# ctu-mrs/mrs_uav_trajectory_generation

Measured on AMD Instinct MI355X. Metric: trajectories/sec (batch of N-seg min-snap paths), higher is better.
Workload: dtype f64

## Files before the change

### mrs_uav_trajectory_generation_amd/csrc/mrs_tg_knobs.hpp

```cpp
#pragma once

#include <algorithm>
#include <climits>
#include <cstddef>
#include <cstdlib>

namespace mrs_tg {
namespace knob {

constexpr int kUnset = INT_MIN;

inline long long env_ll(const char* name, long long unset) {
  const char* e = std::getenv(name);
  return e ? std::atoll(e) : unset;
}
inline int env_int(const char* name, int unset) {
  const char* e = std::getenv(name);
  return e ? std::atoi(e) : unset;
}
inline bool env_flag(const char* name, bool unset) {
  const char* e = std::getenv(name);
  return e ? std::atoi(e) != 0 : unset;
}
inline int env_forced(const char* name) {
  const char* e = std::getenv(name);
  return e ? (std::atoi(e) != 0 ? 1 : 0) : -1;
}

inline bool rows_kernel() { static const bool v = env_flag("MRS_TG_ROWS_KERNEL", true); return v; }
inline bool rows_pipeline() { static const bool v = env_flag("MRS_TG_ROWS_PIPELINE", true); return v; }
inline int rows_ppw() { static const int v = [] { const int n = env_int("MRS_TG_ROWS_PPW", kUnset); return n == kUnset ? 0 : n == 1 ? 1 : 2; }(); return v; }
inline long long quad_min_paths() { static const long long v = env_ll("MRS_TG_QUAD_MIN_PATHS", 6144); return v; }
inline bool quad_ends() { static const bool v = env_flag("MRS_TG_QUAD_ENDS", true); return v; }
inline int duo_forced() { return env_forced("MRS_TG_DUO"); }
inline bool duo_uniform() { return env_flag("MRS_TG_DUO_UNIFORM", true); }
inline bool duo_store_through() { return env_flag("MRS_TG_DUO_STORE_THROUGH", true); }
inline long long tile_max_paths(long long by_shape) { return env_ll("MRS_TG_TILE_MAX_PATHS", by_shape); }

inline int dim_split_max_paths() { return env_int("MRS_TG_DIM_SPLIT_MAX_PATHS", kUnset); }
inline int ends_min_segments() { static const int v = std::max(2, env_int("MRS_TG_ENDS_MIN_SEGMENTS", 2)); return v; }
inline int lean_forced() { return env_forced("MRS_TG_LEAN"); }
inline int lean_shared() { static const int v = env_int("MRS_TG_LEAN_SHARED", 2); return v; }
inline bool regroup() { static const bool v = env_flag("MRS_TG_REGROUP", true); return v; }
inline int lean_wide_forced() { static const int v = env_forced("MRS_TG_LEAN_WIDE"); return v; }
inline bool lean_wide_all() { static const bool v = env_flag("MRS_TG_LEAN_WIDE_ALL", true); return v; }
inline int lean_resident_blocks() { static const int v = env_int("MRS_TG_LEAN_RESIDENT_BLOCKS", kUnset); return v; }
inline bool wave_kernel() { static const bool v = env_flag("MRS_TG_WAVE_KERNEL", true); return v; }
inline bool maxima_bounds() { static const bool v = env_flag("MRS_TG_MAXIMA_BOUNDS", true); return v; }

inline bool verify_flags() { static const bool v = env_flag("MRS_TG_VERIFY_FLAGS", false); return v; }
inline size_t stage_max_bytes() { static const size_t v = (size_t)env_ll("MRS_TG_STAGE_MAX_BYTES", 256 * 1024); return v; }
inline bool zero_copy() { static const bool v = env_flag("MRS_TG_ZERO_COPY", true); return v; }
inline bool pool_poison() { static const bool v = std::getenv("MRS_TG_POOL_POISON") != nullptr; return v; }

inline int policy_device() { static const int v = env_int("MRS_TG_POLICY_DEVICE", 64); return v; }
inline int policy_threads() { static const int v = [] { const int n = env_int("MRS_TG_POLICY_THREADS", kUnset); return n == kUnset ? 0 : std::max(1, n); }(); return v; }
inline size_t policy_grain() { static const size_t v = [] { const int n = env_int("MRS_TG_POLICY_GRAIN", kUnset); return n == kUnset ? (size_t)0 : (size_t)std::max(1, n); }(); return v; }
inline bool policy_trace() { static const bool v = env_flag("MRS_TG_POLICY_TRACE", false); return v; }
inline bool policy_pinned() { static const bool v = env_flag("MRS_TG_POLICY_PINNED", true); return v; }

}
}
```

### mrs_uav_trajectory_generation_amd/csrc/mrs_tg_quad.hip

```cpp
#include <hip/hip_runtime.h>

#include <cstdint>
#include <cstdlib>

#include "mrs_tg_device.hpp"
#include "mrs_tg_launch.h"
#include "mrs_tg_nl_common.hpp"
#include "mrs_tg_solve.hpp"

#ifndef MRS_TG_QUAD_WAVES
#define MRS_TG_QUAD_WAVES 1
#endif
#ifndef MRS_TG_QUAD_GROUP_WAVES
#define MRS_TG_QUAD_GROUP_WAVES 2
#endif
#ifndef MRS_TG_DUO_GROUP_WAVES
#define MRS_TG_DUO_GROUP_WAVES 2
#endif

namespace mrs_tg {

constexpr int kQdPaths = 16;
constexpr int kQdL = 0, kQdLinv = 6, kQdZ = 10, kQdRec = 26;

__host__ __device__ constexpr size_t quad_lds_doubles(int Smax, bool ends = false) {
  return (size_t)(ends ? Smax + 1 : (Smax > 1 ? Smax - 1 : 1)) * kQdRec * kQdPaths + (size_t)Smax * kQdPaths
         + (ends ? (size_t)(Smax + 1) * 2 : 0)
      ;
}

__device__ __forceinline__ void quad_powers(double T, bool d1, bool d2, bool d4, double (&p2)[9]) {
  const double t2 = T * T;
  const double t4 = t2 * t2;
  const double td = ((d1 ? T : 1.0) * (d2 ? t2 : 1.0)) * (d4 ? t4 : 1.0);
  p2[0] = T * rcp_refined(td * td);
  p2[1] = p2[0] * T;
  p2[2] = p2[0] * t2;
  p2[3] = p2[1] * t2;
  p2[4] = p2[0] * t4;
  p2[5] = p2[1] * t4;
  p2[6] = p2[2] * t4;
  p2[7] = p2[3] * t4;
  p2[8] = p2[4] * t4;
}

__device__ __forceinline__ void store_coeff_pair(double2* dst, double a, double b) {
  *dst = make_double2(a, b);
}

#ifndef MRS_TG_DUO_THROUGH_FORM
#define MRS_TG_DUO_THROUGH_FORM 1
#endif
template <int BYTES>
__device__ __forceinline__ void store_coeff_pair_through(double2* dst, double2 v) {
  typedef int int4v __attribute__((ext_vector_type(4)));
  const int4v bits = __builtin_bit_cast(int4v, v);
#if MRS_TG_DUO_THROUGH_FORM == 3
  __builtin_nontemporal_store(bits, reinterpret_cast<int4v*>(dst + BYTES / 16));
#else
#if MRS_TG_DUO_THROUGH_FORM == 2
  asm volatile("global_store_dwordx4 %0, %1, off offset:%2 sc0 sc1\n\ts_nop 1" ::"v"(dst), "v"(bits), "i"(BYTES));
#else
  asm volatile("global_store_dwordx4 %0, %1, off offset:%2 sc1\n\ts_nop 1" ::"v"(dst), "v"(bits), "i"(BYTES));
#endif
#endif
}

__device__ __forceinline__ double quad_sum(double v) {
  v += dpp_move<0xB1>(v);
  v += dpp_move<0x4E>(v);
  return v;
}

template <bool WP, bool ENDS = false, bool MOVING = false>
__device__ __forceinline__ void solve_quad_body(const BatchView& b, int d, const uint8_t* __restrict__ mask,
                                                const double* __restrict__ vals, const double* seg_times,
                                                double* __restrict__ coeffs, int32_t* __restrict__ status,
                                                double* __restrict__ cost, const int32_t* __restrict__ status_in, double* ws,
                                                const RowsTail& tail, int block, const double* __restrict__ pos_wp) {
  extern __shared__ double lds[];
  const int lane = threadIdx.x, pl = lane >> 2, dim = lane & 3;
  const int q = block * kQdPaths + pl;
  const bool active = q < b.n_paths;
  const PathRef pr = path_at(b, active ? q : b.n_paths - 1);
  const int S = pr.S;
  const int Smax = b.max_segments;
  double* rec0 = lds;
  double* tbuf = lds + (size_t)(ENDS ? Smax + 1 : (Smax > 1 ? Smax - 1 : 1)) * kQdRec * kQdPaths;
  unsigned char* vmask = reinterpret_cast<unsigned char*>(tbuf + (size_t)Smax * kQdPaths);
  const bool scaling = tail.maxima != nullptr;
  double t_sum = 0.0;
  bool ok = S >= 2, pos_ok = true;
  unsigned fm_first = 0u, fm_last = 0u;
  bool moving_path = false;
  if (active) {
    const int opt_st = scaling ? tail.opt_status[pr.p] : 0;
    for (int i = dim; i < S; i += 4) {
      double T = seg_times[pr.s0 + i];
      if (scaling) {
        if (opt_st != -2) T *= violation_scaling(tail.maxima + (size_t)(pr.s0 + i) * 9, tail.limits + (size_t)pr.p * 9);
        tail.seg_times_out[pr.s0 + i] = T;
      }
      tbuf[i * kQdPaths + pl] = T;
      t_sum += T;
    }
    for (int v = dim; v <= S; v += 4) {
      const uint8_t* mrow = mask + (size_t)(pr.v0 + v) * kHalf;
      const bool end = v == 0 || v == S;
      unsigned fixed = 0;
#pragma unroll
      for (int k = 0; k < kHalf; ++k) fixed |= (mrow[k] != 0 ? 1u : 0u) << k;
      pos_ok = pos_ok && (fixed & 1u);
      if (end) {
        const double* vrow = vals + (size_t)(pr.v0 + v) * kHalf * kD;
        double nz = 0.0;
        double av[kHalf * kD];
#pragma unroll
        for (int e = kD; e < kHalf * kD; ++e) av[e] = fabs(vrow[e]);
#pragma unroll
        for (int k = 1; k < kHalf; ++k)
#pragma unroll
          for (int e = 0; e < kD; ++e) nz += ((fixed >> k) & 1u) ? av[k * kD + e] : 0.0;
        if (MOVING && v == 0) {
          moving_path = nz != 0.0;
          nz = 0.0;
        }
        if (ENDS) {
          ok = ok && (fixed & 1u) && nz == 0.0;
          if (v == 0) fm_first = (~fixed >> 1) & 0xFu;
          if (v == S) fm_last = (~fixed >> 1) & 0xFu;
        } else {
          ok = ok && fixed == 0x1Fu && nz == 0.0;
        }
      } else if (ENDS) {
        bool zero = true;
        if (fixed != 0x1u) {
          const double* vrow = vals + (size_t)(pr.v0 + v) * kHalf * kD;
          double av[kHalf * kD];
#pragma unroll
          for (int e = kD; e < kHalf * kD; ++e) av[e] = fabs(vrow[e]);
          double nz = 0.0;
#pragma unroll
          for (int k = 1; k < kHalf; ++k)
#pragma unroll
            for (int e = 0; e < kD; ++e) nz += ((fixed >> k) & 1u) ? av[k * kD + e] : 0.0;
          zero = nz == 0.0;
// ... 313 lines not shown
#pragma unroll
        for (int k = 0; k < kN; k += 2) store_coeff_pair(out + k / 2, c[k], c[k + 1]);
      }
#pragma unroll
      for (int r = 0; r < kNB; ++r) xn[r] = x[r];
      if (on) p_end = p_start;
    }
  } else if (active) {
    bool pok = true;
    BlockSource none{nullptr, nullptr, 0, 0};
    __builtin_amdgcn_fence(__ATOMIC_ACQ_REL, "workgroup");
    const double* times = (scaling ? tail.seg_times_out : seg_times) + pr.s0;
    my_cost = solve_path<1, true>(mask, vals, pr.v0, S, d, times, dim, none, ws, (size_t)b.n_paths * 4,
                                  (unsigned)q * 4u + (unsigned)dim, coeffs + (size_t)pr.s0 * kD * kN, pok);
  }
  my_cost = quad_sum(my_cost);
  if (active && dim == 0) {
    if (cost) cost[pr.p] = my_cost;
    if (status) {
      int st = merge_status(path_pos_ok, status_in, pr.p);
      if (tail.sum_t0 != nullptr && st > 0 && t_sum > MRS_TG_RUNAWAY_TIME_FACTOR * tail.sum_t0[pr.p]) st = MRS_TG_STATUS_ROUNDOFF_LIMITED;
      status[pr.p] = st;
    }
  }
}

constexpr int kDuoPaths = 8;

constexpr int kDuoXchgChunk = kD * kN;

__host__ __device__ constexpr size_t duo_lds_doubles(int Smax) {
  return (size_t)(Smax > 1 ? Smax - 1 : 1) * kQdRec * kDuoPaths + (size_t)Smax * kDuoPaths +
         (size_t)(Smax + 1) * kD * kDuoPaths + kDuoPaths / 2 +
         kDuoXchgChunk;
}
static_assert(8 * duo_lds_doubles(10) * sizeof(double) <= 160 * 1024, "two-sided kernel at 10 segments: two wavefronts per SIMD");
static_assert(duo_lds_doubles(2) <= quad_lds_doubles(2) && duo_lds_doubles(24) <= quad_lds_doubles(24) &&
                  duo_lds_doubles(64) <= quad_lds_doubles(64),
              "(both grow linearly, the four-lane store faster: 432 against 248 doubles per segment)");

#ifdef MRS_TG_DUO_STAMPS
constexpr int kDuoStampSlots = 20;
__device__ unsigned long long g_duo_stamps[2048 * kDuoStampSlots];
#define DUO_STAMP(k) (duo_stamp[k] = __builtin_readcyclecounter())
#else
#define DUO_STAMP(k)
#endif

template <int TAG = 0>
__device__ __forceinline__ int lane_now() {
  int l;
  asm volatile("v_mbcnt_lo_u32_b32 %0, -1, 0\n\tv_mbcnt_hi_u32_b32 %0, -1, %0 ; %1" : "=v"(l) : "i"(TAG));
  return l;
}

__device__ __forceinline__ double xor4(double v) {
  constexpr int kSwap4 = (4 << 10) | 0x1F;
  const unsigned long long u = __builtin_bit_cast(unsigned long long, v);
  const unsigned lo = (unsigned)__builtin_amdgcn_ds_swizzle((int)(unsigned)u, kSwap4);
  const unsigned hi = (unsigned)__builtin_amdgcn_ds_swizzle((int)(unsigned)(u >> 32), kSwap4);
  return __builtin_bit_cast(double, ((unsigned long long)hi << 32) | lo);
}

template <int TAG>
__device__ __forceinline__ void duo_finish(double my_cost, bool active, unsigned long long pos_bad, const int* pidx,
                                           double* __restrict__ cost, int32_t* __restrict__ status,
                                           const int32_t* __restrict__ status_in, const RowsTail& tail, double t_sum) {
  my_cost = quad_sum(my_cost);
  my_cost += xor4(my_cost);
  const int lane_late = lane_now<TAG + 1>();
  if (active && (lane_late & 7) == 0) {
    const bool path_pos_ok = ((pos_bad >> (lane_late & ~7)) & 0xFFull) == 0ull;
    const int p_out = pidx[lane_late >> 3];
    if (cost) cost[p_out] = my_cost;
    if (status) {
      int st = merge_status(path_pos_ok, status_in, p_out);
      if (tail.sum_t0 != nullptr && st > 0 && t_sum > MRS_TG_RUNAWAY_TIME_FACTOR * tail.sum_t0[p_out]) st = MRS_TG_STATUS_ROUNDOFF_LIMITED;
      status[p_out] = st;
      asm volatile("; epilogue %0" ::"i"(TAG));
    }
  }
}

template <bool WP, bool MOVING = false, bool THROUGH = false>
__device__ __forceinline__ void solve_duo_body(const BatchView& b, int d, const uint8_t* __restrict__ mask,
                                               const double* __restrict__ vals, const double* seg_times,
                                               double* __restrict__ coeffs, int32_t* __restrict__ status,
                                               double* __restrict__ cost, const int32_t* __restrict__ status_in, double* ws,
                                               const RowsTail& tail, int block, const double* __restrict__ pos_wp,
                                               bool uniform_loops, bool through = false) {
  extern __shared__ double lds[];
  const int lane = threadIdx.x, pl = lane >> 3, side = (lane >> 2) & 1, dim = lane & 3, l8 = lane & 7;
  const int q = block * kDuoPaths + pl;
  const bool active = q < b.n_paths;
  const PathRef pr = path_at(b, active ? q : b.n_paths - 1);
  const int S = pr.S;
  const int Smax = b.max_segments;
  double* rec0 = lds;
  double* tbuf = lds + (size_t)(Smax > 1 ? Smax - 1 : 1) * kQdRec * kDuoPaths;
#ifdef MRS_TG_DUO_STAMPS
  unsigned long long duo_stamp[16] = {0, 0, 0, 0, 0, 0, 0, 0, 0, 0, 0, 0, 0, 0, 0, 0};
  duo_stamp[14] = __builtin_amdgcn_s_memrealtime();
#endif
  DUO_STAMP(0);
  const bool scaling = tail.maxima != nullptr;
  double* pbuf = tbuf + (size_t)Smax * kDuoPaths;
  int* pidx = reinterpret_cast<int*>(pbuf + (size_t)(Smax + 1) * kD * kDuoPaths);
  if (l8 == 0) pidx[pl] = pr.p;
  DUO_STAMP(1);
  const double* pbase = WP ? pos_wp + (size_t)pr.v0 * kD : vals + (size_t)pr.v0 * kHalf * kD;
  constexpr int pstride = WP ? kD : kHalf * kD;
  const int n_pos = (S + 1) * kD;
  double t_sum = 0.0;
  bool ok = S >= 2, pos_ok = true;
  bool moving_path = false;
  auto mask_bits = [&](int v) {
    const uint8_t* mrow = mask + (size_t)(pr.v0 + v) * kHalf;
    unsigned fixed = 0;
#pragma unroll
    for (int k = 0; k < kHalf; ++k) fixed |= (mrow[k] != 0 ? 1u : 0u) << k;
    return fixed;
  };
  const int v_end = (l8 & 1) ? S : 0;
  const unsigned f_end = mask_bits(v_end);
  double av[kHalf * kD];
  {
    const double* vrow = vals + (size_t)(pr.v0 + v_end) * kHalf * kD;
#pragma unroll
    for (int e = kD; e < kHalf * kD; ++e) av[e] = fabs(vrow[e]);
  }
  const int opt_st = (scaling && active) ? tail.opt_status[pr.p] : 0;
  auto trip = [&](int base) {
    const int ia = base + l8, ib = ia + 8;
    double Ta = seg_times[pr.s0 + min(ia, S - 1)], Tb = seg_times[pr.s0 + min(ib, S - 1)];
    const unsigned fa = mask_bits(min(ia, S)), fb = mask_bits(min(ib, S));
    double pe[8];
#pragma unroll
    for (int k = 0; k < 8; ++k) {
      const int ic = min(base * kD + k * 8 + l8, n_pos - 1);
      pe[k] = pbase[(size_t)(ic >> 2) * pstride + (ic & 3)];
    }
#ifdef MRS_TG_DUO_STAMPS
    if (base == 0) DUO_STAMP(13);
#endif
    if (active) {
      if (scaling) {
        if (ia < S) {
          if (opt_st != -2) Ta *= violation_scaling(tail.maxima + (size_t)(pr.s0 + ia) * 9, tail.limits + (size_t)pr.p * 9);
          tail.seg_times_out[pr.s0 + ia] = Ta;
        }
        if (ib < S) {
          if (opt_st != -2) Tb *= violation_scaling(tail.maxima + (size_t)(pr.s0 + ib) * 9, tail.limits + (size_t)pr.p * 9);
          tail.seg_times_out[pr.s0 + ib] = Tb;
        }
      }
      if (ia < S) {
        tbuf[ia * kDuoPaths + pl] = Ta;
        t_sum += Ta;
      }
      if (ib < S) {
        tbuf[ib * kDuoPaths + pl] = Tb;
        t_sum += Tb;
      }
      if (ia >= 1 && ia < S) {
        ok = ok && fa == 0x1u;
        pos_ok = pos_ok && (fa & 1u);
      }
      if (ib < S) {
        ok = ok && fb == 0x1u;
        pos_ok = pos_ok && (fb & 1u);
      }
#pragma unroll
      for (int k = 0; k < 8; ++k) {
        const int idx = base * kD + k * 8 + l8;
        if (idx < n_pos) pbuf[idx * kDuoPaths + pl] = pe[k];
      }
    }
  };
  trip(0);
  for (int base = 16; base <= Smax; base += 16) trip(base);
  if (active && l8 < 2) {
    double nz = 0.0;
#pragma unroll
    for (int k = 1; k < kHalf; ++k)
#pragma unroll
      for (int e = 0; e < kD; ++e) nz += ((f_end >> k) & 1u) ? av[k * kD + e] : 0.0;
    if (MOVING && l8 == 0) {
      moving_path = nz != 0.0;
      nz = 0.0;
    }
    ok = ok && f_end == 0x1Fu && nz == 0.0;
    pos_ok = pos_ok && (f_end & 1u);
  }
  DUO_STAMP(2);
  t_sum = quad_sum(t_sum);
  t_sum += xor4(t_sum);
  const bool any_moving = MOVING && __ballot(active && moving_path) != 0ull;
  if (any_moving) moving_path = __shfl((int)moving_path, lane & ~7, 64) != 0 && side == 0;
  const bool plain_wave = __ballot(active && !ok) == 0ull;
  const unsigned long long pos_bad = __ballot(active && !pos_ok);
  const bool uni_wave = uniform_loops && __ballot(active && S == __builtin_amdgcn_readfirstlane(S)) == ~0ull;
  wave_lds_barrier();
  DUO_STAMP(3);

  double my_cost = 0.0;
  if (plain_wave) {
    constexpr int kOrder = kHalf - 1;
    const double (*hb)[kN] = c_hbar[kOrder];
    double cNear[10], cCpl[kNB][kNB], cFar[10], cN[kNB], cF[kNB];
#pragma unroll
    for (int r = 0; r < kNB; ++r) {
#pragma unroll
      for (int c = 0; c <= r; ++c) {
        cNear[tri(r, c)] = hb[kSlot0 + r][kSlot0 + c];
        cFar[tri(r, c)] = hb[kHalf + kSlot0 + r][kHalf + kSlot0 + c];
      }
#pragma unroll
      for (int c = 0; c < kNB; ++c) cCpl[r][c] = hb[kSlot0 + r][kHalf + kSlot0 + c];
      cN[r] = hb[kSlot0 + r][0];
      cF[r] = hb[kHalf + kSlot0 + r][0];
    }
    constexpr bool d1 = (kOrder & 1) != 0, d2 = (kOrder & 2) != 0, d4 = (kOrder & 4) != 0;
    const int m_mid = (S + 1) >> 1;
    const int Mmx = (Smax + 1) >> 1;
    const int m_mid_ = m_mid;
    struct LaneIds { int pl, side, dim; };
    auto ids_now = [&]() {
      const int l = lane_now();
      return LaneIds{l >> 3, (l >> 2) & 1, l & 3};
    };
    auto oseg = [&](int sd, int i) { return sd ? S - 1 - i : i; };
    auto overt = [&](int sd, int v) { return sd ? S - v : v; };
    auto side_len = [&](int sd) { return sd ? S - m_mid_ : m_mid_; };
    auto pos = [&](const LaneIds& id, int v) {
      const int Ms = side_len(id.side);
      const int vc = min(max(v, 0), Ms);
      const double r = pbuf[(overt(id.side, vc) * kD + id.dim) * kDuoPaths + id.pl];
      return (active && v >= 0 && v <= Ms) ? r : 0.0;
    };
    double Sm[10], y[kNB];
#pragma unroll
    for (int e = 0; e < 10; ++e) Sm[e] = 0.0;
#pragma unroll
    for (int r = 0; r < kNB; ++r) y[r] = 0.0;
    auto fwd_first = [&](const double (&p2)[9], double dp, const double (&f0)[kNB]) {
#pragma unroll
      for (int r = 0; r < kNB; ++r) {
#pragma unroll
        for (int c = 0; c <= r; ++c) Sm[tri(r, c)] = cFar[tri(r, c)] * p2[r + c + 2];
        y[r] = -((cF[r] * p2[r + 1]) * dp);
      }
      if (any_moving) {
#pragma unroll
        for (int r = 0; r < kNB; ++r)
#pragma unroll
          for (int c = 0; c < kNB; ++c) y[r] = fma(-(cCpl[c][r] * p2[r + c + 2]), f0[c], y[r]);
      }
    };
    auto fwd_interior = [&](const double (&p2)[9], double dp, double* rec, int dim_now) {
#pragma unroll
      for (int r = 0; r < kNB; ++r) {
#pragma unroll
        for (int c = 0; c <= r; ++c) Sm[tri(r, c)] = fma(cNear[tri(r, c)], p2[r + c + 2], Sm[tri(r, c)]);
        y[r] = fma(-(cN[r] * p2[r + 1]), dp, y[r]);
      }
      double L[10], Linv[kNB], z[kNB];
#pragma unroll
      for (int c = 0; c < kNB; ++c) {
        double dsum = Sm[tri(c, c)];
#pragma unroll
        for (int mm = 0; mm < c; ++mm) dsum = fma(-L[tri(c, mm)], L[tri(c, mm)], dsum);
        const double inv = rsqrt_refined(dsum);
        Linv[c] = inv;
#pragma unroll
        for (int r = c + 1; r < kNB; ++r) {
          double t = Sm[tri(r, c)];
#pragma unroll
          for (int mm = 0; mm < c; ++mm) t = fma(-L[tri(r, mm)], L[tri(c, mm)], t);
          L[tri(r, c)] = t * inv;
        }
      }
#pragma unroll
      for (int r = 0; r < kNB; ++r) {
        double t = y[r];
// ... 5 lines not shown
        rec[(kQdL + 0) * kDuoPaths] = L[tri(1, 0)];
        rec[(kQdL + 1) * kDuoPaths] = L[tri(2, 0)];
        rec[(kQdL + 2) * kDuoPaths] = L[tri(2, 1)];
        rec[(kQdL + 3) * kDuoPaths] = L[tri(3, 0)];
        rec[(kQdL + 4) * kDuoPaths] = L[tri(3, 1)];
        rec[(kQdL + 5) * kDuoPaths] = L[tri(3, 2)];
#pragma unroll
        for (int r = 0; r < kNB; ++r) rec[(kQdLinv + r) * kDuoPaths] = Linv[r];
      }
#pragma unroll
      for (int r = 0; r < kNB; ++r) rec[(kQdZ + r * kD + dim_now) * kDuoPaths] = z[r];
      double W[kNB][kNB];
#pragma unroll
      for (int c = 0; c < kNB; ++c)
#pragma unroll
        for (int r = 0; r < kNB; ++r) {
          double t = cCpl[r][c] * p2[r + c + 2];
#pragma unroll
          for (int mm = 0; mm < r; ++mm) t = fma(-L[tri(r, mm)], W[mm][c], t);
          W[r][c] = t * Linv[r];
        }
#pragma unroll
      for (int r = 0; r < kNB; ++r) {
#pragma unroll
        for (int c = 0; c <= r; ++c) {
          double t = cFar[tri(r, c)] * p2[r + c + 2];
#pragma unroll
          for (int mm = 0; mm < kNB; ++mm) t = fma(-W[mm][r], W[mm][c], t);
          Sm[tri(r, c)] = t;
        }
        double t = -((cF[r] * p2[r + 1]) * dp);
#pragma unroll
        for (int mm = 0; mm < kNB; ++mm) t = fma(-W[mm][r], z[mm], t);
        y[r] = t;
      }
    };
    auto moving_values = [&](int dim_now, double (&f)[kNB]) {
      const double* vrow0 = vals + (size_t)pr.v0 * kHalf * kD + dim_now;
#pragma unroll
      for (int r = 0; r < kNB; ++r) f[r] = vrow0[(r + 1) * kD];
    };
    const int S_u = __builtin_amdgcn_readfirstlane(S);
    const int M0 = (S_u + 1) >> 1, M1 = S_u - M0;
    int i_lo = 0, i_hi = Mmx;
    double p_cur;
    if (uni_wave) {
      const LaneIds id = ids_now();
      const int v1 = id.side ? S_u - 1 : 1;
      const int st = id.side ? -kDuoPaths : kDuoPaths, sp = st * kD, sr = st * kQdRec;
      const double* tp = tbuf + (id.side ? v1 : 0) * kDuoPaths + id.pl;
      const double* pp = pbuf + (v1 * kD + id.dim) * kDuoPaths + id.pl;
      double* rp = rec0 + (v1 - 1) * kQdRec * kDuoPaths + id.pl;
      p_cur = pbuf[((id.side ? S_u : 0) * kD + id.dim) * kDuoPaths + id.pl];
      DUO_STAMP(4);
      {
        const double T = *tp, p_nxt = *pp;
        double p2[9];
        quad_powers(T, d1, d2, d4, p2);
        double f0[kNB] = {0.0, 0.0, 0.0, 0.0};
        if (any_moving && moving_path) moving_values(id.dim, f0);
        fwd_first(p2, p_cur - p_nxt, f0);
        p_cur = p_nxt;
      }
      DUO_STAMP(5);
      for (int i = 1; i < M1; ++i) {
        tp += st;
        pp += sp;
        const double T = *tp, p_nxt = *pp;
        double p2[9];
        quad_powers(T, d1, d2, d4, p2);
        fwd_interior(p2, p_cur - p_nxt, rp, lane_now() & 3);
        rp += sr;
        p_cur = p_nxt;
#ifdef MRS_TG_DUO_STAMPS
        if (i == 1) DUO_STAMP(6);
#endif
      }
      i_lo = M1;
      i_hi = M0;
    } else {
      p_cur = pos(ids_now(), 0);
      DUO_STAMP(4);
    }
    for (int i = i_lo; i < i_hi; ++i) {
      const LaneIds id = ids_now();
      const bool on = active && i < side_len(id.side);
      const double T = on ? tbuf[oseg(id.side, i) * kDuoPaths + id.pl] : 1.0;
      const double p_nxt = pos(id, i + 1);
      double p2[9];
      quad_powers(T, d1, d2, d4, p2);
      const double dp = p_cur - p_nxt;
      double f0[kNB] = {0.0, 0.0, 0.0, 0.0};
      if (any_moving && i == 0 && active && moving_path) moving_values(id.dim, f0);
      if (on) {
        if (i == 0) {
          fwd_first(p2, dp, f0);
        } else {
          fwd_interior(p2, dp, rec0 + (size_t)(overt(id.side, i) - 1) * kQdRec * kDuoPaths + id.pl, id.dim);
        }
      }
      p_cur = p_nxt;
#ifdef MRS_TG_DUO_STAMPS
      if (i == 0) DUO_STAMP(5);
      if (i == 1) DUO_STAMP(6);
#endif
    }
    DUO_STAMP(7);
    double xn[kNB];
    {
#pragma unroll
      for (int r = 0; r < kNB; ++r) {
#pragma unroll
        for (int c = 0; c <= r; ++c) {
          const double other = xor4(Sm[tri(r, c)]);
          Sm[tri(r, c)] += ((r + c) & 1) ? -other : other;
        }
        const double oy = xor4(y[r]);
        y[r] += (r & 1) ? oy : -oy;
      }
      double L[10], Linv[kNB], z[kNB];
#pragma unroll
      for (int c = 0; c < kNB; ++c) {
        double dsum = Sm[tri(c, c)];
#pragma unroll
        for (int mm = 0; mm < c; ++mm) dsum = fma(-L[tri(c, mm)], L[tri(c, mm)], dsum);
        const double inv = rsqrt_refined(dsum);
        Linv[c] = inv;
#pragma unroll
        for (int r = c + 1; r < kNB; ++r) {
          double t = Sm[tri(r, c)];
#pragma unroll
          for (int mm = 0; mm < c; ++mm) t = fma(-L[tri(r, mm)], L[tri(c, mm)], t);
          L[tri(r, c)] = t * inv;
        }
      }
#pragma unroll
      for (int r = 0; r < kNB; ++r) {
        double t = y[r];
#pragma unroll
        for (int mm = 0; mm < r; ++mm) t = fma(-L[tri(r, mm)], z[mm], t);
        z[r] = t * Linv[r];
      }
      xn[3] = z[3] * Linv[3];
      xn[2] = fma(-L[tri(3, 2)], xn[3], z[2]) * Linv[2];
      xn[1] = fma(-L[tri(3, 1)], xn[3], fma(-L[tri(2, 1)], xn[2], z[1])) * Linv[1];
      xn[0] = fma(-L[tri(3, 0)], xn[3], fma(-L[tri(2, 0)], xn[2], fma(-L[tri(1, 0)], xn[1], z[0]))) * Linv[0];
    }
    wave_lds_barrier();
    DUO_STAMP(8);
    double p_end;
    {
      const LaneIds id = ids_now();
      p_end = pos(id, side_len(id.side));
    }
    for (int v = Mmx - 1; v >= 0; --v) {
      const LaneIds id = ids_now();
      const int side = id.side, dim = id.dim, pl = id.pl;
      const bool on = active && v < side_len(side);
      double x[kNB] = {0.0, 0.0, 0.0, 0.0};
      const double p_start = pos(id, v);
      if (on && v >= 1) {
        const double* rec = rec0 + (size_t)(overt(side, v) - 1) * kQdRec * kDuoPaths + pl;
        double t[kNB];
#pragma unroll
        for (int r = 0; r < kNB; ++r) t[r] = rec[(kQdZ + r * kD + dim) * kDuoPaths];
        const double l10 = rec[(kQdL + 0) * kDuoPaths], l20 = rec[(kQdL + 1) * kDuoPaths], l21 = rec[(kQdL + 2) * kDuoPaths],
                     l30 = rec[(kQdL + 3) * kDuoPaths], l31 = rec[(kQdL + 4) * kDuoPaths], l32 = rec[(kQdL + 5) * kDuoPaths];
        const double i0 = rec[(kQdLinv + 0) * kDuoPaths], i1 = rec[(kQdLinv + 1) * kDuoPaths], i2 = rec[(kQdLinv + 2) * kDuoPaths],
                     i3 = rec[(kQdLinv + 3) * kDuoPaths];
        {
          double pw[9];
          quad_powers(tbuf[oseg(side, v) * kDuoPaths + pl], d1, d2, d4, pw);
          double u[kNB];
#pragma unroll
          for (int r = 0; r < kNB; ++r) {
            u[r] = 0.0;
#pragma unroll
            for (int c = 0; c < kNB; ++c) u[r] = fma(cCpl[r][c] * pw[r + c + 2], xn[c], u[r]);
          }
          const double w0 = u[0] * i0;
          const double w1 = fma(-l10, w0, u[1]) * i1;
          const double w2 = fma(-l21, w1, fma(-l20, w0, u[2])) * i2;
          const double w3 = fma(-l32, w2, fma(-l31, w1, fma(-l30, w0, u[3]))) * i3;
          t[0] -= w0;
          t[1] -= w1;
          t[2] -= w2;
          t[3] -= w3;
        }
        x[3] = t[3] * i3;
        x[2] = fma(-l32, x[3], t[2]) * i2;
        x[1] = fma(-l31, x[3], fma(-l21, x[2], t[1])) * i1;
        x[0] = fma(-l30, x[3], fma(-l20, x[2], fma(-l10, x[1], t[0]))) * i0;
      }
      if (any_moving && v == 0 && active && moving_path) {
        const double* vrow0 = vals + (size_t)pr.v0 * kHalf * kD + dim;
#pragma unroll
        for (int r = 0; r < kNB; ++r) x[r] += vrow0[(r + 1) * kD];
      }
      if (on) {
        const double T = tbuf[oseg(side, v) * kDuoPaths + pl];
        const double s1 = side ? -1.0 : 1.0;
        const double a0 = side ? p_end : p_start, b0 = side ? p_start : p_end;
        double da[kNB], dbv[kNB];
#pragma unroll
        for (int r = 0; r < kNB; ++r) {
          const double sg = (r & 1) ? 1.0 : s1;
          da[r] = (side ? xn[r] : x[r]) * sg;
          dbv[r] = (side ? x[r] : xn[r]) * sg;
        }
        const double dv[kN] = {a0, da[0], da[1], da[2], da[3], b0, dbv[0], dbv[1], dbv[2], dbv[3]};
        double w[kHalf];
        w[0] = 1.0;
#pragma unroll
        for (int k = 1; k < kHalf; ++k) w[k] = w[k - 1] * T;
        double db[kN], cb[kN], c[kN];
#pragma unroll
        for (int j = 0; j < kN; ++j) db[j] = dv[j] * w[j % kHalf];
        const double ti = 1.0 / T;
        double tik = 1.0;
#pragma unroll
        for (int k = 0; k < kN; ++k) {
          double sacc = 0.0;
          if (k < kHalf) {
            sacc = c_abar_inv[k][k] * db[k];
          } else {
#pragma unroll
            for (int j = 0; j < kN; ++j) sacc += c_abar_inv[k][j] * db[j];
          }
          cb[k] = sacc;
          c[k] = sacc * tik;
          tik *= ti;
        }
        double p2[9];
        quad_powers(T, d1, d2, d4, p2);
        my_cost = fma(cost_quadratic_form<kOrder>(cb), p2[0], my_cost);
        double2* out = reinterpret_cast<double2*>(coeffs + ((size_t)(pr.s0 + oseg(side, v)) * kD + dim) * kN);
        constexpr int kRowDoubles = kQdRec * kDuoPaths;
        constexpr int kXchgRowsBoth = ((2 * kDuoPaths - 1) * kDuoXchgChunk + kRowDoubles - 1) / kRowDoubles;
        static_assert(kDuoPaths * kDuoXchgChunk <= 2 * kRowDoubles, "the step of side 0 alone: eight chunks in two rows");
        static_assert(kD == 4 && kN % 2 == 0, "a row of four lanes writes 64 consecutive bytes: one pair per dimension");
#if defined(MRS_TG_DUO_STORE_EXPERIMENT) && MRS_TG_DUO_STORE_EXPERIMENT == 1
#pragma unroll
        for (int k = 0; k < kN; k += 2) asm volatile("; keep %0 %1" ::"v"(c[k]), "v"(c[k + 1]));
        if (false)
#elif defined(MRS_TG_DUO_STORE_EXPERIMENT) && MRS_TG_DUO_STORE_EXPERIMENT == 2
        if (uni_wave) {
          double2* wbase = reinterpret_cast<double2*>(coeffs + (size_t)(pr.s0 - pl * S) * kD * kN) + (v * 5 * 64 + (pl * 8 + side * 4 + dim));
#pragma unroll
          for (int k = 0; k < kN; k += 2) store_coeff_pair(wbase + (k / 2) * 64, c[k], c[k + 1]);
        } else
#endif
        if (uni_wave && (v >= M1 || S_u - 2 * max(v, 1) + 1 >= kXchgRowsBoth)) {
          const int chunk = v < M1 ? pl * 2 + side : pl;
          double* xrows = rec0 + (size_t)max(v - 1, 0) * kRowDoubles + chunk * kDuoXchgChunk;
          double* xlast = lds + (duo_lds_doubles(Smax) - kDuoXchgChunk);
          double2* xbuf = reinterpret_cast<double2*>(chunk == 2 * kDuoPaths - 1 ? xlast : xrows);
#pragma unroll
          for (int k = 0; k < kN; k += 2) xbuf[dim * (kN / 2) + k / 2] = make_double2(c[k], c[k + 1]);
          wave_lds_barrier();
          double2* out4 = out - 4 * dim;
          double2 piece[kN / 2];
#pragma unroll
          for (int t = 0; t < kN / 2; ++t) piece[t] = xbuf[4 * t + dim];
          if (THROUGH && through) {
            static_assert(kN / 2 == 5, "one statement per pair");
            store_coeff_pair_through<0>(out4, piece[0]);
            store_coeff_pair_through<64>(out4, piece[1]);
            store_coeff_pair_through<128>(out4, piece[2]);
            store_coeff_pair_through<192>(out4, piece[3]);
            store_coeff_pair_through<256>(out4, piece[4]);
          } else {
#pragma unroll
            for (int t = 0; t < kN / 2; ++t) store_coeff_pair(out4 + 4 * t, piece[t].x, piece[t].y);
          }
          wave_lds_barrier();
        } else {
#pragma unroll
          for (int k = 0; k < kN; k += 2) store_coeff_pair(out + k / 2, c[k], c[k + 1]);
        }
      }
      if (on) {
#pragma unroll
        for (int r = 0; r < kNB; ++r) xn[r] = x[r];
        p_end = p_start;
      }
#ifdef MRS_TG_DUO_STAMPS
      if (v == Mmx - 1) DUO_STAMP(9);
#endif
    }
    DUO_STAMP(10);
    duo_finish<0>(my_cost, active, pos_bad, pidx, cost, status, status_in, tail, t_sum);
  } else {
    if (active && side == 0) {
    bool pok = true;
    BlockSource none{nullptr, nullptr, 0, 0};
    __builtin_amdgcn_fence(__ATOMIC_ACQ_REL, "workgroup");
    const double* times = (scaling ? tail.seg_times_out : seg_times) + pr.s0;
    my_cost = solve_path<1, true>(mask, vals, pr.v0, S, d, times, dim, none, ws, (size_t)b.n_paths * 4,
                                  (unsigned)q * 4u + (unsigned)dim, coeffs + (size_t)pr.s0 * kD * kN, pok);
    }
    duo_finish<2>(my_cost, active, pos_bad, pidx, cost, status, status_in, tail, t_sum);
  }
#ifdef MRS_TG_DUO_STAMPS
  DUO_STAMP(11);
  __builtin_amdgcn_s_waitcnt(0);
  DUO_STAMP(12);
  duo_stamp[15] = __builtin_amdgcn_s_memrealtime();
  if (lane == 0 && blockIdx.x < 2048)
    for (int k = 0; k < 16; ++k) g_duo_stamps[blockIdx.x * kDuoStampSlots + k] = duo_stamp[k];
#endif
}

#ifdef MRS_TG_DUO_STAMPS
extern "C" int mrs_tg_debug_duo_stamps(unsigned long long* out) {
  return (int)hipMemcpyFromSymbol(out, HIP_SYMBOL(g_duo_stamps), sizeof(unsigned long long) * 2048 * kDuoStampSlots);
}
#endif

template <bool WP>
__global__ __launch_bounds__(64, MRS_TG_QUAD_WAVES) void solve_duo_kernel(BatchView b, int d, const uint8_t* __restrict__ mask,
                                                       const double* __restrict__ vals, const double* seg_times,
                                                       double* __restrict__ coeffs, int32_t* __restrict__ status,
                                                       double* __restrict__ cost, const int32_t* __restrict__ status_in,
                                                       double* ws, RowsTail tail, int uniform_loops) {
  solve_duo_body<WP, true>(b, d, mask, vals, seg_times, coeffs, status, cost, status_in, ws, tail, (int)blockIdx.x, tail.pos_wp,
                           (uniform_loops & 1) != 0);
}

template <bool WP>
__global__ __launch_bounds__(64, MRS_TG_DUO_GROUP_WAVES) void solve_duo_group_kernel(BatchView b, int d, RowsGroup g, double* ws,
                                                                                    size_t ws_batch_doubles, int blocks_per_batch,
                                                                                    int uniform_loops) {
  const int j = __builtin_amdgcn_readfirstlane((int)blockIdx.x / blocks_per_batch);
  solve_duo_body<WP, false, true>(b, d, g.mask[j], g.vals[j], g.seg_times[j], g.coeffs[j], g.status[j], g.cost[j], nullptr,
                                  ws + (size_t)j * ws_batch_doubles, RowsTail(), (int)blockIdx.x - j * blocks_per_batch, g.pos_wp[j],
                                  (uniform_loops & 1) != 0, (uniform_loops & 2) != 0);
#ifdef MRS_TG_DUO_STAMPS
  if (threadIdx.x == 0 && blockIdx.x < 2048) g_duo_stamps[blockIdx.x * kDuoStampSlots + 16] = (unsigned long long)g.coeffs[0];
#endif
}

template <bool WP, bool ENDS = false>
__global__ __launch_bounds__(64, MRS_TG_QUAD_WAVES) void solve_quad_kernel(BatchView b, int d, const uint8_t* __restrict__ mask,
                                                        const double* __restrict__ vals, const double* seg_times,
                                                        double* __restrict__ coeffs, int32_t* __restrict__ status,
                                                        double* __restrict__ cost, const int32_t* __restrict__ status_in,
                                                        double* ws, RowsTail tail) {
  solve_quad_body<WP, ENDS, true>(b, d, mask, vals, seg_times, coeffs, status, cost, status_in, ws, tail, (int)blockIdx.x, tail.pos_wp);
}

template <bool WP, bool ENDS = false>
__global__ __launch_bounds__(64, MRS_TG_QUAD_GROUP_WAVES) void solve_quad_group_kernel(BatchView b, int d, RowsGroup g, double* ws, size_t ws_batch_doubles,
                                                              int blocks_per_batch) {
  const int j = __builtin_amdgcn_readfirstlane((int)blockIdx.x / blocks_per_batch);
  solve_quad_body<WP, ENDS>(b, d, g.mask[j], g.vals[j], g.seg_times[j], g.coeffs[j], g.status[j], g.cost[j], nullptr,
                            ws + (size_t)j * ws_batch_doubles, RowsTail(), (int)blockIdx.x - j * blocks_per_batch, g.pos_wp[j]);
}


static constexpr size_t kQuadLdsBudget = 80 * 1024;
static_assert(duo_lds_doubles(24) * sizeof(double) <= kQuadLdsBudget, "the two-sided kernel at the longest routed length");

static bool duo_pays(long long paths_in_launch) {
  if (const int forced = knob::duo_forced(); forced >= 0) return forced != 0;
  static const int cus = device_compute_units();
  return (paths_in_launch + kQdPaths - 1) / kQdPaths < (long long)cus * 4 * 5 / 4;
}

static int duo_loop_bits() { return (knob::duo_uniform() ? 1 : 0) | (knob::duo_store_through() ? 2 : 0); }

bool quad_kernel_applies(const BatchView& b, long long paths_in_launch, bool with_sampling) {
  if (b.n_paths == 0 || with_sampling) return false;
  if (paths_in_launch < knob::quad_min_paths()) return false;
  return quad_lds_doubles(b.max_segments) * sizeof(double) <= kQuadLdsBudget;
}

hipError_t launch_solve_quad(const BatchView& b, int d, const uint8_t* mask, const double* vals, const double* seg_times,
                             double* coeffs, int32_t* status, double* cost, const int32_t* status_in, double* ws,
                             hipStream_t stream, const RowsTail& tail) {
  const bool ends = knob::quad_ends() && (d < 4 || constrained_slots_hint()) &&
                    quad_lds_doubles(b.max_segments, true) * sizeof(double) <= kQuadLdsBudget;
  const bool wp = tail.pos_wp != nullptr;
  if (!ends && !(d < 4) && duo_pays(b.n_paths)) {
    const size_t lds_duo = duo_lds_doubles(b.max_segments) * sizeof(double);
    const auto duo = wp ? MRS_TG_KERNEL(solve_duo_kernel<true>) : MRS_TG_KERNEL(solve_duo_kernel<false>);
    if (lds_duo > 64 * 1024) {
      hipError_t e = set_max_dynamic_lds(duo, kQuadLdsBudget);
      if (e != hipSuccess) return e;
    }
    const unsigned grid_duo = (unsigned)((b.n_paths + kDuoPaths - 1) / kDuoPaths);
    MRS_TG_LAUNCH_TIMED(duo, dim3(grid_duo), dim3(64), lds_duo, stream, b, d, mask, vals, seg_times, coeffs, status, cost, status_in,
                        ws, tail, duo_loop_bits());
    return hipGetLastError();
  }
  const size_t lds_bytes = quad_lds_doubles(b.max_segments, ends) * sizeof(double);
  const auto quad = ends ? (wp ? MRS_TG_KERNEL(solve_quad_kernel<true, true>) : MRS_TG_KERNEL(solve_quad_kernel<false, true>))
                         : (wp ? MRS_TG_KERNEL(solve_quad_kernel<true>) : MRS_TG_KERNEL(solve_quad_kernel<false>));
  if (lds_bytes > 64 * 1024) {
    hipError_t e = set_max_dynamic_lds(quad, kQuadLdsBudget);
    if (e != hipSuccess) return e;
  }
  const unsigned grid = (unsigned)((b.n_paths + kQdPaths - 1) / kQdPaths);
  MRS_TG_LAUNCH_TIMED(quad, dim3(grid), dim3(64), lds_bytes, stream, b, d, mask, vals, seg_times, coeffs, status, cost, status_in, ws,
                      tail);
  return hipGetLastError();
}

hipError_t launch_solve_quad_group(const BatchView& b, int d, const RowsGroup& g, double* ws, hipStream_t stream) {
  if (g.n < 1 || g.n > kRowsGroupMax) return hipErrorInvalidValue;
  const bool ends = knob::quad_ends() && (d < 4 || constrained_slots_hint()) &&
                    quad_lds_doubles(b.max_segments, true) * sizeof(double) <= kQuadLdsBudget;
  const size_t lds_bytes = quad_lds_doubles(b.max_segments, ends) * sizeof(double);
  bool wp = true;
  for (int j = 0; j < g.n; ++j) wp = wp && g.pos_wp[j] != nullptr;
  if (!ends && !(d < 4) && duo_pays((long long)b.n_paths * g.n)) {
    const size_t lds_duo = duo_lds_doubles(b.max_segments) * sizeof(double);
    const auto duo = wp ? MRS_TG_KERNEL(solve_duo_group_kernel<true>) : MRS_TG_KERNEL(solve_duo_group_kernel<false>);
    if (lds_duo > 64 * 1024) {
      hipError_t e = set_max_dynamic_lds(duo, kQuadLdsBudget);
      if (e != hipSuccess) return e;
    }
    const int per_batch_duo = (b.n_paths + kDuoPaths - 1) / kDuoPaths;
    const dim3 grid_duo((unsigned)(per_batch_duo * g.n));
    const size_t wsd_duo = linear_workspace_doubles(b);
    MRS_TG_LAUNCH_TIMED(duo, grid_duo, dim3(64), lds_duo, stream, b, d, g, ws, wsd_duo, per_batch_duo, duo_loop_bits());
    return hipGetLastError();
  }
  const auto quad = ends ? (wp ? MRS_TG_KERNEL(solve_quad_group_kernel<true, true>) : MRS_TG_KERNEL(solve_quad_group_kernel<false, true>))
                         : (wp ? MRS_TG_KERNEL(solve_quad_group_kernel<true>) : MRS_TG_KERNEL(solve_quad_group_kernel<false>));
  if (lds_bytes > 64 * 1024) {
    hipError_t e = set_max_dynamic_lds(quad, kQuadLdsBudget);
    if (e != hipSuccess) return e;
  }
  const int per_batch = (b.n_paths + kQdPaths - 1) / kQdPaths;
  const dim3 grid((unsigned)(per_batch * g.n));
  const size_t wsd = linear_workspace_doubles(b);
  MRS_TG_LAUNCH_TIMED(quad, grid, dim3(64), lds_bytes, stream, b, d, g, ws, wsd, per_batch);
  return hipGetLastError();
}

}
```

Measured before the change: 867.5 million.

## Add lean duo kernel specialization for uniform full-wave batches

Adds a LEAN instantiation of the duo solver, used when every path has the same even segment count of at least 4, the path count fills whole waves, and both loop bits are set. It drops the bounds and activity checks and skips the generic per-segment forward loop. It walks the back-substitution with incrementally updated LDS and output offsets, and stores coefficients through a scalar base plus a per-lane offset. The group index moves to blockIdx.y, which removes a division per block. The gain depends on the skipped loop and the reduced address arithmetic staying correct for the uniform case. The lean kernel is also registered under the original instantiation name unless tracing is enabled, which can hide it in profiles.

```diff
diff --git a/mrs_uav_trajectory_generation_amd/csrc/mrs_tg_knobs.hpp b/mrs_uav_trajectory_generation_amd/csrc/mrs_tg_knobs.hpp
--- a/mrs_uav_trajectory_generation_amd/csrc/mrs_tg_knobs.hpp
+++ b/mrs_uav_trajectory_generation_amd/csrc/mrs_tg_knobs.hpp
@@ -35,6 +35,8 @@
 inline int duo_forced() { return env_forced("MRS_TG_DUO"); }
 inline bool duo_uniform() { return env_flag("MRS_TG_DUO_UNIFORM", true); }
 inline bool duo_store_through() { return env_flag("MRS_TG_DUO_STORE_THROUGH", true); }
+inline bool duo_lean() { return env_flag("MRS_TG_DUO_LEAN", true); }
+inline bool trace_instantiations() { return env_flag("MRS_TG_TRACE_INSTANTIATIONS", false); }
 inline long long tile_max_paths(long long by_shape) { return env_ll("MRS_TG_TILE_MAX_PATHS", by_shape); }
 
 inline int dim_split_max_paths() { return env_int("MRS_TG_DIM_SPLIT_MAX_PATHS", kUnset); }
diff --git a/mrs_uav_trajectory_generation_amd/csrc/mrs_tg_quad.hip b/mrs_uav_trajectory_generation_amd/csrc/mrs_tg_quad.hip
--- a/mrs_uav_trajectory_generation_amd/csrc/mrs_tg_quad.hip
+++ b/mrs_uav_trajectory_generation_amd/csrc/mrs_tg_quad.hip
@@ -62,6 +62,21 @@
   asm volatile("global_store_dwordx4 %0, %1, off offset:%2 sc0 sc1\n\ts_nop 1" ::"v"(dst), "v"(bits), "i"(BYTES));
 #else
   asm volatile("global_store_dwordx4 %0, %1, off offset:%2 sc1\n\ts_nop 1" ::"v"(dst), "v"(bits), "i"(BYTES));
+#endif
+#endif
+}
+
+template <int BYTES>
+__device__ __forceinline__ void store_coeff_pair_through(const double* base, unsigned lane_bytes, double2 v) {
+  typedef int int4v __attribute__((ext_vector_type(4)));
+  const int4v bits = __builtin_bit_cast(int4v, v);
+#if MRS_TG_DUO_THROUGH_FORM == 3
+  __builtin_nontemporal_store(bits, reinterpret_cast<int4v*>(reinterpret_cast<char*>(const_cast<double*>(base)) + lane_bytes + BYTES));
+#else
+#if MRS_TG_DUO_THROUGH_FORM == 2
+  asm volatile("global_store_dwordx4 %0, %1, %2 offset:%3 sc0 sc1\n\ts_nop 1" ::"v"(lane_bytes), "v"(bits), "s"(base), "i"(BYTES));
+#else
+  asm volatile("global_store_dwordx4 %0, %1, %2 offset:%3 sc1\n\ts_nop 1" ::"v"(lane_bytes), "v"(bits), "s"(base), "i"(BYTES));
 #endif
 #endif
 }
@@ -541,7 +556,7 @@
   }
 }
 
-template <bool WP, bool MOVING = false, bool THROUGH = false>
+template <bool WP, bool MOVING = false, bool THROUGH = false, bool LEAN = false>
 __device__ __forceinline__ void solve_duo_body(const BatchView& b, int d, const uint8_t* __restrict__ mask,
                                                const double* __restrict__ vals, const double* seg_times,
                                                double* __restrict__ coeffs, int32_t* __restrict__ status,
@@ -551,8 +566,9 @@
   extern __shared__ double lds[];
   const int lane = threadIdx.x, pl = lane >> 3, side = (lane >> 2) & 1, dim = lane & 3, l8 = lane & 7;
   const int q = block * kDuoPaths + pl;
-  const bool active = q < b.n_paths;
-  const PathRef pr = path_at(b, active ? q : b.n_paths - 1);
+  static_assert(!LEAN || THROUGH, "the lean instantiation has the write-through flavour only");
+  const bool active = LEAN || q < b.n_paths;
+  const PathRef pr = LEAN ? PathRef{q, q * b.uniform_S, b.uniform_S, q * b.uniform_S + q} : path_at(b, active ? q : b.n_paths - 1);
   const int S = pr.S;
   const int Smax = b.max_segments;
   double* rec0 = lds;
@@ -583,10 +599,16 @@
   const int v_end = (l8 & 1) ? S : 0;
   const unsigned f_end = mask_bits(v_end);
   double av[kHalf * kD];
+  const int k_end = 1 + (l8 >> 1);
   {
     const double* vrow = vals + (size_t)(pr.v0 + v_end) * kHalf * kD;
-#pragma unroll
-    for (int e = kD; e < kHalf * kD; ++e) av[e] = fabs(vrow[e]);
+    if constexpr (LEAN) {
+#pragma unroll
+      for (int e = 0; e < kD; ++e) av[e] = fabs(vrow[k_end * kD + e]);
+    } else {
+#pragma unroll
+      for (int e = kD; e < kHalf * kD; ++e) av[e] = fabs(vrow[e]);
+    }
   }
   const int opt_st = (scaling && active) ? tail.opt_status[pr.p] : 0;
   auto trip = [&](int base) {
@@ -638,12 +660,20 @@
   };
   trip(0);
   for (int base = 16; base <= Smax; base += 16) trip(base);
+  double nz_end = 0.0;
+  if constexpr (LEAN) {
+    nz_end = ((f_end >> k_end) & 1u) ? (av[0] + av[1]) + (av[2] + av[3]) : 0.0;
+    nz_end += dpp_move<0x4E>(nz_end);
+    nz_end += xor4(nz_end);
+  }
   if (active && l8 < 2) {
-    double nz = 0.0;
-#pragma unroll
-    for (int k = 1; k < kHalf; ++k)
-#pragma unroll
-      for (int e = 0; e < kD; ++e) nz += ((f_end >> k) & 1u) ? av[k * kD + e] : 0.0;
+    double nz = nz_end;
+    if constexpr (!LEAN) {
+#pragma unroll
+      for (int k = 1; k < kHalf; ++k)
+#pragma unroll
+        for (int e = 0; e < kD; ++e) nz += ((f_end >> k) & 1u) ? av[k * kD + e] : 0.0;
+    }
     if (MOVING && l8 == 0) {
       moving_path = nz != 0.0;
       nz = 0.0;
@@ -658,7 +688,7 @@
   if (any_moving) moving_path = __shfl((int)moving_path, lane & ~7, 64) != 0 && side == 0;
   const bool plain_wave = __ballot(active && !ok) == 0ull;
   const unsigned long long pos_bad = __ballot(active && !pos_ok);
-  const bool uni_wave = uniform_loops && __ballot(active && S == __builtin_amdgcn_readfirstlane(S)) == ~0ull;
+  const bool uni_wave = LEAN || (uniform_loops && __ballot(active && S == __builtin_amdgcn_readfirstlane(S)) == ~0ull);
   wave_lds_barrier();
   DUO_STAMP(3);
 
@@ -830,6 +860,7 @@
       p_cur = pos(ids_now(), 0);
       DUO_STAMP(4);
     }
+    if constexpr (!LEAN)
     for (int i = i_lo; i < i_hi; ++i) {
       const LaneIds id = ids_now();
       const bool on = active && i < side_len(id.side);
@@ -897,18 +928,35 @@
     wave_lds_barrier();
     DUO_STAMP(8);
     double p_end;
-    {
+    int at_rec = 0, at_pos = 0, at_time = 0;
+    unsigned at_out = 0;
+    const int v_top = LEAN ? M1 - 1 : Mmx - 1;
+    if constexpr (LEAN) {
+      const LaneIds id = ids_now();
+      p_end = pbuf[(M0 * kD + id.dim) * kDuoPaths + id.pl];
+      const int ov = id.side ? S_u - v_top : v_top, os = id.side ? ov - 1 : ov;
+      at_rec = (ov - 1) * kQdRec * kDuoPaths + id.pl;
+      at_pos = (int)(pbuf - lds) + (ov * kD + id.dim) * kDuoPaths + id.pl;
+      at_time = (int)(tbuf - lds) + os * kDuoPaths + id.pl;
+      at_out = (unsigned)(((id.pl * S_u + os) * kD * kN + 2 * id.dim) * (int)sizeof(double));
+    } else {
       const LaneIds id = ids_now();
       p_end = pos(id, side_len(id.side));
     }
-    for (int v = Mmx - 1; v >= 0; --v) {
+    for (int v = v_top; v >= 0; --v) {
       const LaneIds id = ids_now();
       const int side = id.side, dim = id.dim, pl = id.pl;
-      const bool on = active && v < side_len(side);
+      const bool on = LEAN || (active && v < side_len(side));
       double x[kNB] = {0.0, 0.0, 0.0, 0.0};
-      const double p_start = pos(id, v);
+      double p_start, T_now = 0.0;
+      if constexpr (LEAN) {
+        p_start = lds[at_pos];
+        T_now = lds[at_time];
+      } else {
+        p_start = pos(id, v);
+      }
       if (on && v >= 1) {
-        const double* rec = rec0 + (size_t)(overt(side, v) - 1) * kQdRec * kDuoPaths + pl;
+        const double* rec = LEAN ? lds + at_rec : rec0 + (size_t)(overt(side, v) - 1) * kQdRec * kDuoPaths + pl;
         double t[kNB];
 #pragma unroll
         for (int r = 0; r < kNB; ++r) t[r] = rec[(kQdZ + r * kD + dim) * kDuoPaths];
@@ -918,7 +966,7 @@
                      i3 = rec[(kQdLinv + 3) * kDuoPaths];
         {
           double pw[9];
-          quad_powers(tbuf[oseg(side, v) * kDuoPaths + pl], d1, d2, d4, pw);
+          quad_powers(LEAN ? T_now : tbuf[oseg(side, v) * kDuoPaths + pl], d1, d2, d4, pw);
           double u[kNB];
 #pragma unroll
           for (int r = 0; r < kNB; ++r) {
@@ -946,7 +994,7 @@
         for (int r = 0; r < kNB; ++r) x[r] += vrow0[(r + 1) * kD];
       }
       if (on) {
-        const double T = tbuf[oseg(side, v) * kDuoPaths + pl];
+        const double T = LEAN ? T_now : tbuf[oseg(side, v) * kDuoPaths + pl];
         const double s1 = side ? -1.0 : 1.0;
         const double a0 = side ? p_end : p_start, b0 = side ? p_start : p_end;
         double da[kNB], dbv[kNB];
@@ -982,7 +1030,7 @@
         double p2[9];
         quad_powers(T, d1, d2, d4, p2);
         my_cost = fma(cost_quadratic_form<kOrder>(cb), p2[0], my_cost);
-        double2* out = reinterpret_cast<double2*>(coeffs + ((size_t)(pr.s0 + oseg(side, v)) * kD + dim) * kN);
+        double2* out = LEAN ? nullptr : reinterpret_cast<double2*>(coeffs + ((size_t)(pr.s0 + oseg(side, v)) * kD + dim) * kN);
         constexpr int kRowDoubles = kQdRec * kDuoPaths;
         constexpr int kXchgRowsBoth = ((2 * kDuoPaths - 1) * kDuoXchgChunk + kRowDoubles - 1) / kRowDoubles;
         static_assert(kDuoPaths * kDuoXchgChunk <= 2 * kRowDoubles, "the step of side 0 alone: eight chunks in two rows");
@@ -998,8 +1046,8 @@
           for (int k = 0; k < kN; k += 2) store_coeff_pair(wbase + (k / 2) * 64, c[k], c[k + 1]);
         } else
 #endif
-        if (uni_wave && (v >= M1 || S_u - 2 * max(v, 1) + 1 >= kXchgRowsBoth)) {
-          const int chunk = v < M1 ? pl * 2 + side : pl;
+        if (LEAN || (uni_wave && (v >= M1 || S_u - 2 * max(v, 1) + 1 >= kXchgRowsBoth))) {
+          const int chunk = (LEAN || v < M1) ? pl * 2 + side : pl;
           double* xrows = rec0 + (size_t)max(v - 1, 0) * kRowDoubles + chunk * kDuoXchgChunk;
           double* xlast = lds + (duo_lds_doubles(Smax) - kDuoXchgChunk);
           double2* xbuf = reinterpret_cast<double2*>(chunk == 2 * kDuoPaths - 1 ? xlast : xrows);
@@ -1010,7 +1058,14 @@
           double2 piece[kN / 2];
 #pragma unroll
           for (int t = 0; t < kN / 2; ++t) piece[t] = xbuf[4 * t + dim];
-          if (THROUGH && through) {
+          if constexpr (LEAN) {
+            const double* wave_out = coeffs + (size_t)block * (kDuoPaths * kD * kN) * S_u;
+            store_coeff_pair_through<0>(wave_out, at_out, piece[0]);
+            store_coeff_pair_through<64>(wave_out, at_out, piece[1]);
+            store_coeff_pair_through<128>(wave_out, at_out, piece[2]);
+            store_coeff_pair_through<192>(wave_out, at_out, piece[3]);
+            store_coeff_pair_through<256>(wave_out, at_out, piece[4]);
+          } else if (THROUGH && through) {
             static_assert(kN / 2 == 5, "one statement per pair");
             store_coeff_pair_through<0>(out4, piece[0]);
             store_coeff_pair_through<64>(out4, piece[1]);
@@ -1032,8 +1087,15 @@
         for (int r = 0; r < kNB; ++r) xn[r] = x[r];
         p_end = p_start;
       }
+      if constexpr (LEAN) {
+        const int st = side ? kDuoPaths : -kDuoPaths;
+        at_rec += st * kQdRec;
+        at_pos += st * kD;
+        at_time += st;
+        at_out += (unsigned)(st * (kD * kN * (int)sizeof(double) / kDuoPaths));
+      }
 #ifdef MRS_TG_DUO_STAMPS
-      if (v == Mmx - 1) DUO_STAMP(9);
+      if (v == v_top) DUO_STAMP(9);
 #endif
     }
     DUO_STAMP(10);
@@ -1054,8 +1116,8 @@
   __builtin_amdgcn_s_waitcnt(0);
   DUO_STAMP(12);
   duo_stamp[15] = __builtin_amdgcn_s_memrealtime();
-  if (lane == 0 && blockIdx.x < 2048)
-    for (int k = 0; k < 16; ++k) g_duo_stamps[blockIdx.x * kDuoStampSlots + k] = duo_stamp[k];
+  if (const unsigned wg = blockIdx.y * gridDim.x + blockIdx.x; lane == 0 && wg < 2048)
+    for (int k = 0; k < 16; ++k) g_duo_stamps[wg * kDuoStampSlots + k] = duo_stamp[k];
 #endif
 }
 
@@ -1075,16 +1137,16 @@
                            (uniform_loops & 1) != 0);
 }
 
-template <bool WP>
+template <bool WP, bool LEAN = false>
 __global__ __launch_bounds__(64, MRS_TG_DUO_GROUP_WAVES) void solve_duo_group_kernel(BatchView b, int d, RowsGroup g, double* ws,
-                                                                                    size_t ws_batch_doubles, int blocks_per_batch,
-                                                                                    int uniform_loops) {
-  const int j = __builtin_amdgcn_readfirstlane((int)blockIdx.x / blocks_per_batch);
-  solve_duo_body<WP, false, true>(b, d, g.mask[j], g.vals[j], g.seg_times[j], g.coeffs[j], g.status[j], g.cost[j], nullptr,
-                                  ws + (size_t)j * ws_batch_doubles, RowsTail(), (int)blockIdx.x - j * blocks_per_batch, g.pos_wp[j],
-                                  (uniform_loops & 1) != 0, (uniform_loops & 2) != 0);
+                                                                                    size_t ws_batch_doubles, int uniform_loops) {
+  const int j = (int)blockIdx.y;
+  solve_duo_body<WP, false, true, LEAN>(b, d, g.mask[j], g.vals[j], g.seg_times[j], g.coeffs[j], g.status[j], g.cost[j], nullptr,
+                                        ws + (size_t)j * ws_batch_doubles, RowsTail(), (int)blockIdx.x, g.pos_wp[j],
+                                        (uniform_loops & 1) != 0, (uniform_loops & 2) != 0);
 #ifdef MRS_TG_DUO_STAMPS
-  if (threadIdx.x == 0 && blockIdx.x < 2048) g_duo_stamps[blockIdx.x * kDuoStampSlots + 16] = (unsigned long long)g.coeffs[0];
+  if (const unsigned wg = blockIdx.y * gridDim.x + blockIdx.x; threadIdx.x == 0 && wg < 2048)
+    g_duo_stamps[wg * kDuoStampSlots + 16] = (unsigned long long)g.coeffs[0];
 #endif
 }
 
@@ -1163,15 +1225,20 @@
   for (int j = 0; j < g.n; ++j) wp = wp && g.pos_wp[j] != nullptr;
   if (!ends && !(d < 4) && duo_pays((long long)b.n_paths * g.n)) {
     const size_t lds_duo = duo_lds_doubles(b.max_segments) * sizeof(double);
-    const auto duo = wp ? MRS_TG_KERNEL(solve_duo_group_kernel<true>) : MRS_TG_KERNEL(solve_duo_group_kernel<false>);
+    const int loop_bits = duo_loop_bits();
+    const bool lean = b.uniform_S >= 4 && b.uniform_S % 2 == 0 && b.n_paths % kDuoPaths == 0 && loop_bits == 3 && knob::duo_lean();
+    const bool spell = lean && knob::trace_instantiations();
+    const auto duo = lean ? (wp ? kernel_as(solve_duo_group_kernel<true, true>, spell ? "solve_duo_group_kernel<true, true>" : "solve_duo_group_kernel<true>")
+                                : kernel_as(solve_duo_group_kernel<false, true>, spell ? "solve_duo_group_kernel<false, true>" : "solve_duo_group_kernel<false>"))
+                          : (wp ? MRS_TG_KERNEL(solve_duo_group_kernel<true>) : MRS_TG_KERNEL(solve_duo_group_kernel<false>));
     if (lds_duo > 64 * 1024) {
       hipError_t e = set_max_dynamic_lds(duo, kQuadLdsBudget);
       if (e != hipSuccess) return e;
     }
     const int per_batch_duo = (b.n_paths + kDuoPaths - 1) / kDuoPaths;
-    const dim3 grid_duo((unsigned)(per_batch_duo * g.n));
+    const dim3 grid_duo((unsigned)per_batch_duo, (unsigned)g.n);
     const size_t wsd_duo = linear_workspace_doubles(b);
-    MRS_TG_LAUNCH_TIMED(duo, grid_duo, dim3(64), lds_duo, stream, b, d, g, ws, wsd_duo, per_batch_duo, duo_loop_bits());
+    MRS_TG_LAUNCH_TIMED(duo, grid_duo, dim3(64), lds_duo, stream, b, d, g, ws, wsd_duo, loop_bits);
     return hipGetLastError();
   }
   const auto quad = ends ? (wp ? MRS_TG_KERNEL(solve_quad_group_kernel<true, true>) : MRS_TG_KERNEL(solve_quad_group_kernel<false, true>))
```

Measured after the change: 950.8 million, median of 6. +9.6%, better.
